# Sukikui/PTI-LDM-VAE

Measured on AMD Instinct MI355X. Metric: vae_train_images_per_sec_256x256, higher is better.
Workload: dtype fp16 forward operands + activations / bf16 backward operands + gradients, fp32 accumulate; 1 GPU; config/vae_dente_no_adv.json 256x256x1 batch 32/GPU: fwd + L1 + 1e-3*KL + bwd + all-reduce + Adam (perceptual term omitted: --perceptual times it; adversarial branch inactive before epoch 6, --adv times it); global_batch=32, parallelism=dp1

## Files before the change

include/pti_vae.h:

```cpp
#ifndef PTI_VAE_H
#define PTI_VAE_H

#include <stdint.h>

#ifdef __cplusplus
extern "C" {
#endif

typedef void* pti_stream_t;

#define PTI_ABI_VERSION 5

#define PTI_OK 0
#define PTI_EINVAL (-1)
#define PTI_EUNSUPPORTED (-2)
#define PTI_ELAUNCH (-3)

#define PTI_CONV_S1 0
#define PTI_CONV_S2PAD 1
#define PTI_CONV_UP2 2
#define PTI_CONV_ZINS 3

#define PTI_PRO_NONE 0
#define PTI_PRO_GN 1
// ... 96 lines not shown
int pti_gn_bwd_blocks(int n, int hw, int c);
int pti_gn_bwd(const void* x, const void* da, const void* dres, void* dx, const int64_t* stats,
               const float* gamma, const float* beta, float* sums, float* partials, float* dgamma,
               float* dbeta, int n, int hw, int c, int groups, float eps, int silu, int x_f16,
               pti_stream_t s);
int pti_conv_gnbwd_tiles(const pti_conv_desc* d);
int pti_conv_gnbwd_chain_supported(int cin, int cout, int ksize);
int pti_conv2d_mfma_gnbwd_chain(const void* g_in, const void* x_in, int x_in_f16, const int64_t* in_stats,
                                const float* in_gamma, const float* in_sums, void* dx_in_out, const void* w_packed,
                                const void* gx, const int64_t* gstats, const float* ggamma, const float* gbeta,
                                void* dy_out, float* gsums, const pti_conv_desc* d, int silu, pti_stream_t s);
int pti_gn_affine_grads(const float* sums, float* dgamma, float* dbeta, int n, int c, pti_stream_t s);
int pti_gn_sums_finalize_affine(const float* partials, float* sums, int n, int tiles, int row_len, const float* affine_sums,
                                float* dgamma, float* dbeta, int affine_c, pti_stream_t s);
int pti_conv2d_mfma_gnbwd(const void* dy_in, const void* w_packed, const void* gx, const int64_t* gstats,
                          const float* ggamma, const float* gbeta, void* dy_out, float* gpartials,
                          const pti_conv_desc* d, int silu, pti_stream_t s);
int pti_gn_sums_finalize(const float* partials, float* sums, int n, int tiles, int row_len,
                         pti_stream_t s);
int pti_gn_bwd_apply(const void* x, const void* dy, const void* dres, void* dx, const int64_t* stats,
                     const float* gamma, const float* beta, const float* sums, float* dgamma,
                     float* dbeta, int n, int hw, int c, int groups, float eps, int x_f16,
                     pti_stream_t s);
int pti_pool2x2_sum(const void* x, void* y, int n, int h, int w, int c, pti_stream_t s);

int pti_attention_fwd(const void* qkv, void* o, float* lse2, int b, int l, int c, pti_stream_t s);
int pti_attention_bwd(const void* qkv, const void* o, const void* dout, const float* lse2,
                      float* delta, void* dqkv, int b, int l, int c, pti_stream_t s);

int pti_latent_head_fwd(const float* h, const float* eps, const float* wm, const float* bm,
                        const float* wl, const float* bl, const float* wp, const float* bp,
                        float* mu, float* sigma, float* logvar, float* zq, int b, int hw, int l,
                        pti_stream_t s);
int pti_post_quant(const float* z_nchw, const float* wp, const float* bp, float* zq_nhwc, int b,
                   int hw, int l, pti_stream_t s);
#define PTI_POST_QUANT_BWD_MAX_BLOCKS 256
#define PTI_POST_QUANT_BWD_WS_FLOATS(l) (PTI_POST_QUANT_BWD_MAX_BLOCKS * ((l) * (l) + (l)))
int pti_post_quant_bwd(const float* dzq_nhwc, const float* z_nchw, const float* wp, float* dz_nchw,
                       float* gwp, float* gbp, float* workspace, int b, int hw, int l,
                       pti_stream_t s);
#define PTI_LATENT_BWD_MAX_BLOCKS 512
#define PTI_LATENT_BWD_WS_FLOATS(l) (PTI_LATENT_BWD_MAX_BLOCKS * 3 * ((l) * (l) + (l)))
int pti_latent_head_bwd(const float* h, const float* eps, const float* wm, const float* bm,
                        const float* wl, const float* bl, const float* wp, const float* bp,
                        const float* dzq, const float* dmu, const float* dsigma, float* dh,
                        float* gwm, float* gbm, float* gwl, float* gbl, float* gwp, float* gbp,
// ... 125 lines not shown
```

pti_ldm_vae_amd/_lib.py:

```python
from __future__ import annotations

import ctypes as C
import os

_HERE = os.path.dirname(os.path.abspath(__file__))
LIB_PATH = os.environ.get("PTI_VAE_LIB") or os.path.join(_HERE, "libpti_vae_hip.so")

def env_overrides() -> dict:
    return {k: v for k, v in sorted(os.environ.items()) if k.startswith("PTI_")}


def refuse_wrong_result_env(who: str) -> None:
    bad = [k for k in os.environ if k.startswith("PTI_") and ("DIAG" in k or k == "PTI_ALLOW_WRONG_RESULTS")]
    if bad:
        raise SystemExit(f"{who}: refusing to run with wrong-result diagnostic variable(s) set: {sorted(bad)} "
                         "(timing diagnostics live in tools/diag_skip.py)")


ABI_VERSION = 5
PTI_CONV_S1, PTI_CONV_S2PAD, PTI_CONV_UP2, PTI_CONV_ZINS = 0, 1, 2, 3
PTI_PRO_NONE, PTI_PRO_GN, PTI_PRO_GN_SILU = 0, 1, 2


class ConvDesc(C.Structure):
# ... 51 lines not shown
    "pti_gn_stats": (_I, [_P, _P, _I, _I, _I, _I, _I, _P]),
    "pti_conv2d_mfma": (_I, [_P, _P, _P, _P, _P, _P, _P, _P, _P, C.POINTER(ConvDesc), _P]),
    "pti_conv2d_mfma_saveact": (_I, [_P, _P, _P, _P, _P, _P, _P, _P, _P, _P, C.POINTER(ConvDesc), _P]),
    "pti_conv2d_direct": (_I, [_P, _P, _P, _P, _P, _P, _P, C.POINTER(ConvDesc), _P]),
    "pti_wgrad_direct": (_I, [_P, _P, _P, _P, _P, _P, _P, _P, _I, _I, _I, _I, _I, _I, _I, _I, _I, _F, _I, _I,
                              C.POINTER(_I64), _I64, _I64, _I64, _P, _I64, _P]),
    "pti_conv_wgrad_workspace_bytes": (_I64, [_I, _I, _I, _I]),
    "pti_conv_wgrad_mfma": (_I, [_P, _P, _P, _P, _P, _P, _P, _P, _I64, _I, C.POINTER(ConvDesc), _P]),
    "pti_conv_wgrad_mfma_partials": (_I, [_P, _P, _P, _P, _P, _P, _I64, C.POINTER(ConvDesc), C.POINTER(_I), _P]),
    "pti_conv_wgrad_mfma_batched": (_I, [C.POINTER(WgradJob), _I, _P, _I64, _P]),
    "pti_conv_wgrad_batched_mode": (_I, [_I, _I, _I, _I, _I]),
    "pti_direct_repack": (_I, [C.POINTER(DirectRepackTable), _P]),
    "pti_conv_wgrad_reduce": (_I, [_P, _I, _P, _P, _I, C.POINTER(ConvDesc), _P]),
    "pti_gn_bwd_blocks": (_I, [_I, _I, _I]),
    "pti_gn_bwd": (_I, [_P, _P, _P, _P, _P, _P, _P, _P, _P, _P, _P, _I, _I, _I, _I, _F, _I, _I, _P]),
    "pti_conv_gnbwd_tiles": (_I, [C.POINTER(ConvDesc)]),
    "pti_gn_sums_finalize": (_I, [_P, _P, _I, _I, _I, _P]),
    "pti_conv2d_mfma_gnbwd": (_I, [_P, _P, _P, _P, _P, _P, _P, _P, C.POINTER(ConvDesc), _I, _P]),
    "pti_conv_gnbwd_chain_supported": (_I, [_I, _I, _I]),
    "pti_conv2d_mfma_gnbwd_chain": (_I, [_P, _P, _I, _P, _P, _P, _P, _P, _P, _P, _P, _P, _P, _P, C.POINTER(ConvDesc), _I, _P]),
    "pti_gn_affine_grads": (_I, [_P, _P, _P, _I, _I, _P]),
    "pti_gn_sums_finalize_affine": (_I, [_P, _P, _I, _I, _I, _P, _P, _P, _I, _P]),
    "pti_gn_bwd_apply": (_I, [_P, _P, _P, _P, _P, _P, _P, _P, _P, _P, _I, _I, _I, _I, _F, _I, _P]),
    "pti_pool2x2_sum": (_I, [_P, _P, _I, _I, _I, _I, _P]),
    "pti_attention_fwd": (_I, [_P, _P, _P, _I, _I, _I, _P]),
    "pti_attention_bwd": (_I, [_P, _P, _P, _P, _P, _P, _I, _I, _I, _P]),
    "pti_latent_head_fwd": (_I, [_P] * 12 + [_I, _I, _I, _P]),
    "pti_post_quant": (_I, [_P, _P, _P, _P, _I, _I, _I, _P]),
    "pti_post_quant_bwd": (_I, [_P, _P, _P, _P, _P, _P, _P, _I, _I, _I, _P]),
    "pti_latent_head_bwd": (_I, [_P] * 19 + [_I, _I, _I, _P]),
    "pti_vae_loss": (_I, [_P, _P, _I64, _P, _P, _I64, _I, _P, _P, _P, _P, _P, _I, _I, _F, _P]),
    "pti_ar_vae_loss": (_I, [_P, _I, _I, _I, _P, _P, _P, _I, _P, _F, _P, _P, _P, _P]),
    "pti_pd_im2col_image": (_I, [_P, _P, _I, _I, _I, _P]),
    "pti_pd_im2col": (_I, [_P, _P, _P, _I, _I, _I, _I, _I, _I, _F, _P]),
    "pti_pd_in_stats": (_I, [_P, _P, _I, _I, _I, _F, _P]),
    "pti_pd_col2im_blocks": (_I, [_I, _I, _I]),
    "pti_pd_col2im": (_I, [_P, _P, _P, _P, _P, _I, _I, _I, _I, _I, _F, _P]),
    "pti_pd_col2im_image": (_I, [_P, _P, _I, _I, _I, _F, _I, _P]),
    "pti_pd_in_bwd_apply": (_I, [_P, _P, _P, _P, _P, _I, _I, _I, _P]),
    "pti_pd_lsgan_blocks": (_I, [_I]),
    "pti_pd_lsgan": (_I, [_P, _I, _I, _I, _F, _F, _F, _P, _P, _P]),
    "pti_pd_final_fwd": (_I, [_P, _P, _P, _P, _P, _I, _I, _I, _I, _F, _P]),
    "pti_pd_final_dgrad": (_I, [_P, _P, _P, _P, _P, _P, _I, _I, _I, _I, _F, _P]),
    "pti_pd_final_wgrad_blocks": (_I, [_I, _I, _I]),
    "pti_pd_final_wgrad": (_I, [_P, _P, _P, _P, _I, _I, _I, _I, _F, _P]),
    "pti_lpips_tap_blocks": (_I, [_I, _I]),
# ... 77 lines not shown
```

pti_ldm_vae_amd/csrc/groupnorm.hip:

```cpp
#include "pti_common.h"

namespace {

__global__ __launch_bounds__(256) void gn_stats_kernel(const bf16* __restrict__ x, stat_t* __restrict__ stats,
                                                       int HW, int C, int G, int pix_per_block, int x_f16) {
  extern __shared__ stat_t sm_q[];
  stat_t* sm = sm_q;
  const int n = blockIdx.y;
  const int tid = threadIdx.x;
  const int NC = C / 8;
  const int ppi = 256 / NC;
  const int lc = tid % NC, lp = tid / NC;
  for (int i = tid; i < 2 * G; i += 256) sm[i] = 0;
  __syncthreads();
  const int p0 = blockIdx.x * pix_per_block;
  const int p1 = min(p0 + pix_per_block, HW);
  float s[8], q[8];
#pragma unroll
  for (int j = 0; j < 8; ++j) s[j] = q[j] = 0.f;
  const bf16* base = x + (size_t)n * HW * C + lc * 8;
  int p = p0 + lp;
  for (; p + 3 * ppi < p1; p += 4 * ppi) {
    u32x4 r[4];
#pragma unroll
// ... 62 lines not shown
  int bps = cdiv(2048, n);
  int ppb = cdiv(hw, bps);
  if (ppb < 16 * ppi) ppb = 16 * ppi;
  ppb = cdiv(ppb, 4 * ppi) * 4 * ppi;
  bps = cdiv(hw, ppb);
  PTI_LAUNCH(gn_stats_kernel, dim3(bps, n), dim3(256), 2 * groups * sizeof(stat_t), (hipStream_t)s,
                     (const bf16*)x, (stat_t*)stats, hw, c, groups, ppb, x_f16);
  PTI_CHECK_LAUNCH("gn_stats");
  return PTI_OK;
}

namespace {

struct GnbArgs {
  const bf16* x; const bf16* da; const bf16* dres; bf16* dx;
  const stat_t* stats; const float* gamma; const float* beta;
  float* sums;
  float* dgamma; float* dbeta;
  int HW, C, G, silu, ppb;
  float eps, inv_cnt;
  int x_f16;
  int N;
  float* part;
};

__global__ __launch_bounds__(256) void gn_bwd_reduce_kernel(GnbArgs a) {
  extern __shared__ float sm[];
  const int n = blockIdx.y, tid = threadIdx.x;
  const int NC = a.C / 8, ppi = 256 / NC, lc = tid % NC, lp = tid / NC;
  for (int i = tid; i < 8 * a.C; i += 256) sm[i] = 0.f;
  __syncthreads();
  const int cpg = a.C / a.G;
  float sc[8], sh[8], mu[8], rs[8];
#pragma unroll
  for (int j = 0; j < 8; ++j) {
    const int ch = lc * 8 + j, g = ch / cpg;
    const float sum = stat_f(a.stats, (n * a.G + g) * 2), sq = stat_f(a.stats, (n * a.G + g) * 2 + 1);
    const float mean = sum * a.inv_cnt;
    const float rstd = rsqrtf(fmaxf(sq * a.inv_cnt - mean * mean, 0.f) + a.eps);
    mu[j] = mean; rs[j] = rstd;
    sc[j] = rstd * a.gamma[ch];
    sh[j] = a.beta[ch] - mean * sc[j];
  }
  float s1[8], s2[8];
#pragma unroll
  for (int j = 0; j < 8; ++j) s1[j] = s2[j] = 0.f;
// ... 67 lines not shown
  if (i < R) {
    const float* p = part + (size_t)n * T * R + i;
    int t = w;
    for (; t + 48 < T; t += 64) {
      const float a0 = p[(size_t)t * R], a1 = p[(size_t)(t + 16) * R], a2 = p[(size_t)(t + 32) * R], a3 = p[(size_t)(t + 48) * R];
      v += (a0 + a1) + (a2 + a3);
    }
    for (; t < T; t += 16) v += p[(size_t)t * R];
  }
  red[w][lane] = v;
  __syncthreads();
  if (w == 0 && i < R) {
    float r[16];
#pragma unroll
    for (int k = 0; k < 16; ++k) r[k] = red[k][lane];
#pragma unroll
    for (int o = 8; o > 0; o >>= 1)
#pragma unroll
      for (int k = 0; k < o; ++k) r[k] += r[k + o];
    sums[(size_t)n * R + i] = r[0];
  }
}

__global__ __launch_bounds__(256) void gn_bwd_apply_kernel(GnbArgs a) {
  const int n = blockIdx.y, tid = threadIdx.x;
  const int NC = a.C / 8, ppi = 256 / NC, lc = tid % NC, lp = tid / NC;
  const int cpg = a.C / a.G;
  const int p0 = blockIdx.x * a.ppb, p1 = min(p0 + a.ppb, a.HW);
  const size_t base = (size_t)n * a.HW * a.C + lc * 8;
  constexpr int U = 4;
  u32x4 rx[U], rd[U], rr[U];
  auto load_batch = [&](int pb) {
#pragma unroll
    for (int u = 0; u < U; ++u) {
      const int p = pb + u * ppi;
      rx[u] = rd[u] = rr[u] = u32x4{0u, 0u, 0u, 0u};
      if (p < p1) {
        rx[u] = __builtin_nontemporal_load((const u32x4*)(a.x + base + (size_t)p * a.C));
        rd[u] = __builtin_nontemporal_load((const u32x4*)(a.da + base + (size_t)p * a.C));
        if (a.dres) rr[u] = __builtin_nontemporal_load((const u32x4*)(a.dres + base + (size_t)p * a.C));
      }
    }
  };
  if (p0 + lp < p1) load_batch(p0 + lp);
  float sc[8], sh[8], mu[8], rs[8], ga[8], c1[8], c2[8];
#pragma unroll
  for (int j = 0; j < 8; ++j) {
    const int ch = lc * 8 + j, g = ch / cpg;
    const float sum = stat_f(a.stats, (n * a.G + g) * 2), sq = stat_f(a.stats, (n * a.G + g) * 2 + 1);
    const float mean = sum * a.inv_cnt;
    const float rstd = rsqrtf(fmaxf(sq * a.inv_cnt - mean * mean, 0.f) + a.eps);
    mu[j] = mean; rs[j] = rstd; ga[j] = a.gamma[ch];
    sc[j] = rstd * ga[j];
    sh[j] = a.beta[ch] - mean * sc[j];
    c1[j] = c2[j] = 0.f;
    if (cpg > 8) {
      float t1 = 0.f, t2 = 0.f;
      for (int cc = g * cpg; cc < (g + 1) * cpg; ++cc) {
        const float gm = a.gamma[cc];
        t1 += gm * a.sums[((size_t)n * a.C + cc) * 2];
        t2 += gm * a.sums[((size_t)n * a.C + cc) * 2 + 1];
      }
      c1[j] = t1 * a.inv_cnt;
      c2[j] = t2 * a.inv_cnt;
    }
  }
  if (cpg <= 8) {
    float w1[8], w2[8];
#pragma unroll
    for (int j = 0; j < 8; ++j) {
      const f32x2 sv = *(const f32x2*)(a.sums + ((size_t)n * a.C + lc * 8 + j) * 2);
      w1[j] = ga[j] * sv[0];
      w2[j] = ga[j] * sv[1];
    }
#pragma unroll
    for (int j = 0; j < 8; ++j) {
      float t1 = 0.f, t2 = 0.f;
#pragma unroll
      for (int jj = 0; jj < 8; ++jj) {
        const bool same = (jj / cpg) == (j / cpg);
        t1 += same ? w1[jj] : 0.f;
        t2 += same ? w2[jj] : 0.f;
      }
      c1[j] = t1 * a.inv_cnt;
      c2[j] = t2 * a.inv_cnt;
    }
  }
  if (blockIdx.x == 0 && n == 0) {
    for (int i = tid; i < a.C; i += 256) {
      float d1 = 0.f, d2 = 0.f;
      for (int m = 0; m < a.N; ++m) {
        d1 += a.sums[((size_t)m * a.C + i) * 2];
        d2 += a.sums[((size_t)m * a.C + i) * 2 + 1];
      }
      if (a.dbeta) a.dbeta[i] += d1;
      if (a.dgamma) a.dgamma[i] += d2;
    }
  }
  for (int pb = p0 + lp; pb < p1; pb += U * ppi) {
    if (pb != p0 + lp) load_batch(pb);
#pragma unroll
    for (int u = 0; u < U; ++u) {
      const int p = pb + u * ppi;
      float fx[8], fd[8], fr[8], o[8];
      unpack8f(rx[u], fx, a.x_f16);
      unpack8(rd[u], fd);
      unpack8(rr[u], fr);
#pragma unroll
      for (int j = 0; j < 8; ++j) {
        float dy = fd[j];
        if (a.silu) dy *= dsilu_f(fx[j] * sc[j] + sh[j]);
// ... 47 lines not shown
  if (n <= 0 || hw <= 0 || c < 8 || (c & (c - 1)) || c > 512) return 0;
  return gn_bwd_grid(n, hw, c, nullptr);
}

extern "C" int pti_gn_bwd(const void* x, const void* da, const void* dres, void* dx, const int64_t* stats,
                          const float* gamma, const float* beta, float* sums, float* partials, float* dgamma,
                          float* dbeta, int n, int hw, int c, int groups, float eps, int silu, int x_f16, pti_stream_t s) {
  if (!x || !da || !dx || !stats || !gamma || !beta || !sums || !partials) PTI_FAIL(PTI_EINVAL, "gn_bwd: null pointer");
  if (c < 8 || c > 512 || (c & (c - 1)) || groups <= 0 || c % groups) PTI_FAIL(PTI_EUNSUPPORTED, "gn_bwd: c=%d groups=%d", c, groups);
  GnbArgs a;
  a.x = (const bf16*)x; a.da = (const bf16*)da; a.dres = (const bf16*)dres; a.dx = (bf16*)dx;
  a.stats = (const stat_t*)stats; a.gamma = gamma; a.beta = beta; a.sums = sums; a.dgamma = dgamma; a.dbeta = dbeta;
  a.HW = hw; a.C = c; a.G = groups; a.silu = silu; a.eps = eps; a.x_f16 = x_f16; a.N = n;
  a.inv_cnt = 1.0f / ((float)(c / groups) * (float)hw);
  int ppb;
  const int bps = gn_bwd_grid(n, hw, c, &ppb);
  a.ppb = ppb;
  a.part = partials;
  PTI_LAUNCH(gn_bwd_reduce_kernel, dim3(bps, n), dim3(256), 8 * c * sizeof(float), (hipStream_t)s, a);
  PTI_CHECK_LAUNCH("gn_bwd_reduce");
  PTI_LAUNCH(gn_sums_finalize_kernel, dim3(cdiv(2 * c, 64), n), dim3(1024), 0, (hipStream_t)s, partials, sums,
                     bps, 2 * c, (const float*)nullptr, (float*)nullptr, (float*)nullptr, 0, 0);
  PTI_CHECK_LAUNCH("gn_sums_finalize");
  PTI_LAUNCH(gn_bwd_apply_kernel, dim3(bps, n), dim3(256), 0, (hipStream_t)s, a);
  PTI_CHECK_LAUNCH("gn_bwd_apply");
  return PTI_OK;
}

extern "C" int pti_gn_bwd_apply(const void* x, const void* dy, const void* dres, void* dx, const int64_t* stats,
                                const float* gamma, const float* beta, const float* sums, float* dgamma, float* dbeta,
                                int n, int hw, int c, int groups, float eps, int x_f16, pti_stream_t s) {
  if (!x || !dy || !dx || !stats || !gamma || !beta || !sums) PTI_FAIL(PTI_EINVAL, "gn_bwd_apply: null pointer");
  if (c < 8 || c > 2048 || (c & (c - 1)) || groups <= 0 || c % groups) PTI_FAIL(PTI_EUNSUPPORTED, "gn_bwd_apply: c=%d groups=%d", c, groups);
  GnbArgs a;
  a.x = (const bf16*)x; a.da = (const bf16*)dy; a.dres = (const bf16*)dres; a.dx = (bf16*)dx;
  a.stats = (const stat_t*)stats; a.gamma = gamma; a.beta = beta; a.sums = const_cast<float*>(sums); a.dgamma = dgamma; a.dbeta = dbeta;
  a.HW = hw; a.C = c; a.G = groups; a.silu = 0; a.eps = eps; a.x_f16 = x_f16; a.N = n;
  a.inv_cnt = 1.0f / ((float)(c / groups) * (float)hw);
  const int ppi = 256 / (c / 8);
  int bps = cdiv(2048, n);
  int ppb = cdiv(hw, bps);
  if (ppb < gnb_min_iters() * ppi) ppb = gnb_min_iters() * ppi;
  ppb = cdiv(ppb, ppi) * ppi;
  bps = cdiv(hw, ppb);
  a.ppb = ppb;
  PTI_LAUNCH(gn_bwd_apply_kernel, dim3(bps, n), dim3(256), 0, (hipStream_t)s, a);
  PTI_CHECK_LAUNCH("gn_bwd_apply");
  return PTI_OK;
}

namespace {
__global__ __launch_bounds__(256) void gn_affine_grads_kernel(const float* __restrict__ sums, float* __restrict__ dgamma,
                                                              float* __restrict__ dbeta, int n, int c) {
  const int i = blockIdx.x * 256 + threadIdx.x;
  if (i >= c) return;
  float d1 = 0.f, d2 = 0.f;
  for (int m = 0; m < n; ++m) {
    const f32x2 sv = *(const f32x2*)(sums + ((size_t)m * c + i) * 2);
    d1 += sv[0];
    d2 += sv[1];
  }
  if (dbeta) dbeta[i] += d1;
  if (dgamma) dgamma[i] += d2;
}
}

extern "C" int pti_gn_affine_grads(const float* sums, float* dgamma, float* dbeta, int n, int c, pti_stream_t s) {
  if (!sums || n <= 0 || c <= 0) PTI_FAIL(PTI_EINVAL, "gn_affine_grads: bad args");
  PTI_LAUNCH(gn_affine_grads_kernel, dim3(cdiv(c, 256)), dim3(256), 0, (hipStream_t)s, sums, dgamma, dbeta, n, c);
  PTI_CHECK_LAUNCH("gn_affine_grads");
// ... 31 lines not shown
```

pti_ldm_vae_amd/engine.py:

```python
from __future__ import annotations

import contextlib
import gc
import os
import warnings

import torch

from . import ops
from .models import autoencoderkl as M
from .ops import (BF16, F32, PTI_CONV_S1, PTI_CONV_S2PAD, PTI_CONV_UP2, PTI_CONV_ZINS, PTI_PRO_GN, PTI_PRO_GN_SILU,
                  PTI_PRO_NONE)


class _Act:

    __slots__ = ("t", "stats")

    def __init__(self, t, stats=None):
        self.t, self.stats = t, stats


def _empty(shape, like, dtype=BF16):
    return torch.empty(shape, dtype=dtype, device=like.device)
# ... 20 lines not shown
                with torch.cuda.graph(g, pool=graphs[0].pool() if graphs else None, capture_error_mode="thread_local"):
                    results.append(body(*results))
                graphs.append(g)
    except Exception as ex:
        warnings.warn(f"HIP-graph capture of {what} failed ({ex!r}); continuing with eager launches")
        torch.cuda.synchronize()
        return None
    return graphs, results


class _MfmaConv:

    def __init__(self, net, wname, bname, ksize, mode, fused_names=None, fwd_f16=True):
        self.net, self.ksize, self.mode = net, ksize, mode
        self.fwd_f16, self.f16 = fwd_f16, False
        self.wname, self.bname, self.fused = wname, bname, fused_names
        if fused_names:
            w0 = net._param_by_name[fused_names[0][0]]
            self.cout, self.cin = 3 * w0.shape[0], w0.shape[1]
        else:
            w = net._param_by_name[wname]
            self.cout, self.cin = w.shape[0], w.shape[1]
        self.wp = self.wpt = None

    def _w(self):
        if self.fused:
            o, n, _ = self.net._slots[self.fused[0][0]]
            return self.net._arena[o:o + 3 * n].view(self.cout, self.cin, 1, 1)
        return self.net._param_by_name[self.wname].data.view(self.cout, self.cin, self.ksize, self.ksize)

    def bias(self):
        if self.fused:
            o, n, _ = self.net._slots[self.fused[0][1]]
            return self.net._arena[o:o + 3 * n]
        return self.net._param_by_name[self.bname].data

    def grads(self):
        if self.fused:
            o, n, _ = self.net._slots[self.fused[0][0]]
            ob, nb, _ = self.net._slots[self.fused[0][1]]
            g = self.net.grad_arena
            return g[o:o + 3 * n], g[ob:ob + 3 * nb]
        return self.net.grad_view(self.wname).view(-1), self.net.grad_view(self.bname)

    def fwd(self, x, *, pro=PTI_PRO_NONE, norm=None, residual=None, want_stats=False, eng=None, act_out=None,
            out_dtype=None):
# ... 2 lines not shown
        y = _empty((n, ho, wo, self.cout), x.t, out_dtype or eng.act_dtype)
        st = eng.new_stats(n) if want_stats else None
        g, b = (norm.weight.data, norm.bias.data) if norm is not None else (None, None)
        ops.conv_mfma(x.t, self.wp, self.bias(), y, cout=self.cout, ksize=self.ksize, mode=self.mode, prologue=pro,
                      in_stats=x.stats if pro else None, gamma=g, beta=b, groups=eng.G, eps=eng.eps,
                      residual=residual, out_stats=st, out_groups=eng.G, act_out=act_out)
        return _Act(y, st)

    def dgrad(self, dy, *, residual=None):
        n, ho, wo, _ = dy.shape
        if self.mode == PTI_CONV_S2PAD:
            out = _empty((n, 2 * ho, 2 * wo, self.cin), dy)
            ops.conv_mfma(dy, self.wpt, None, out, cout=self.cin, ksize=3, mode=PTI_CONV_ZINS, residual=residual)
            return out
        if self.mode == PTI_CONV_UP2:
            pooled = _empty((n, ho // 2, wo // 2, self.cin), dy)
            ops.conv_mfma(dy, self.wpt, None, pooled, cout=self.cin, ksize=self.ksize, mode=PTI_CONV_S1, pool2=True)
            return pooled
        out = _empty((n, ho, wo, self.cin), dy)
        ops.conv_mfma(dy, self.wpt, None, out, cout=self.cin, ksize=self.ksize, mode=PTI_CONV_S1, residual=residual)
        return out

    def dgrad_gn(self, dy, x, norm, *, silu, dres, eng):
        g, sums = self.dgrad_gn_raw(dy, x, norm, silu=silu, eng=eng)
        return self._gn_apply(g, sums, x, norm, dres, eng)

    def _gn_apply(self, g, sums, x, norm, dres, eng):
        dx = _empty(x.t.shape, x.t)
        ops.gn_bwd_apply(x.t, g, dx, x.stats, norm.weight.data, norm.bias.data, sums,
                         norm.net.grad_view(norm.prefix + ".weight"), norm.net.grad_view(norm.prefix + ".bias"),
                         groups=eng.G, eps=eng.eps, dres=dres)
        return dx

    def dgrad_gn_raw(self, dy, x, norm, *, silu, eng):
        n, ho, wo, _ = dy.shape
        g = _empty((n, ho, wo, self.cin), dy)
        sums = eng.zeros(n * self.cin * 2)
        ops.conv_mfma_gnbwd(dy, self.wpt, x.t, x.stats, norm.weight.data, norm.bias.data, g, sums, cout=self.cin,
                            ksize=self.ksize, mode=PTI_CONV_S1, groups=eng.G, eps=eng.eps, silu=silu)
        return g, sums

    def dgrad_gn_chain(self, g_in, x_in, norm_in, sums_in, x, norm, *, silu, dres, eng):
        n, ho, wo, _ = g_in.shape
        dxin = _empty(g_in.shape, g_in)
        dyt = _empty((n, ho, wo, self.cin), g_in)
        sums = eng.zeros(n * self.cin * 2)
# ... 236 lines not shown
        last = len(eb) - 1
        for i in range(1, last - 1):
            self.enc_layers.append(self._make_layer(eb[i], f"encoder.blocks.{i}"))
        self.enc_out = _DirectConv(net, f"encoder.blocks.{last}.conv", norm_prefix=f"encoder.blocks.{last - 1}")
        db = net.decoder.blocks
        self.dec_in = _DirectConv(net, "decoder.blocks.0.conv")
        self.dec_layers = []
        last = len(db) - 1
        for i in range(1, last - 1):
            self.dec_layers.append(self._make_layer(db[i], f"decoder.blocks.{i}"))
        self.dec_out = _DirectConv(net, f"decoder.blocks.{last}.conv", norm_prefix=f"decoder.blocks.{last - 1}")
        self.mfma_convs = [c for l in self.enc_layers + self.dec_layers for c in l.convs]
        for c in self.mfma_convs:
            c.f16 = c.fwd_f16 and self.act_dtype == torch.float16
        self.direct_convs = [self.enc_in, self.enc_out, self.dec_in, self.dec_out]
        self.enc_out.pack_f16 = self.act_dtype == torch.float16
        img = os.environ.get("PTI_IMG_MFMA", "1") == "1"
        self.enc_in.img_mfma = img and 2 <= net.in_channels <= 8 and net.channels[0] % 32 == 0
        self.dec_out.img_mfma = img and 2 <= net.out_channels <= 8 and net.channels[0] % 32 == 0
        self.enc_in.pack_f16 = self.dec_out.pack_f16 = self.act_dtype == torch.float16
        self._wgrad_posts, self._wgrad_zero = [], ()
        self._flush_up = int(os.environ.get("PTI_WGRAD_FLUSH_UP", "1"))
        self.gnbwd_chain = os.environ.get("PTI_GNBWD_CHAIN", "0") == "1"
        self.Lc = net.latent_channels
        self._plist = list(net._param_by_name.values())

    def saves_activated_input(self, t) -> bool:
        return t.shape[1] * t.shape[2] >= self.save_act_min_hw

    def _make_layer(self, blk, prefix):
        if isinstance(blk, M.AEKLResBlock):
            return _ResBlock(self.net, prefix, blk)
        if isinstance(blk, M.AEKLDownsample):
            return _Resample(self.net, prefix + ".conv.conv", PTI_CONV_S2PAD, prefix + ".")
        if isinstance(blk, M.Upsample):
            return _Resample(self.net, prefix + ".postconv.conv", PTI_CONV_UP2, prefix + ".")
        if isinstance(blk, M.SpatialAttentionBlock):
            return _Attention(self.net, prefix)
        raise TypeError(f"unsupported block {type(blk)} at {prefix}")

    def new_stats(self, n):
        return self.zeros(n * self.G * 4).view(torch.int64).view(n, self.G, 2)

    def zeros(self, count):
        count = (count + 3) // 4 * 4
        pool = self._zpool
# ... 459 lines not shown
```

pti_ldm_vae_amd/ops.py:

```python
from __future__ import annotations

import ctypes as C
import os
from collections import namedtuple

import torch

from . import _lib as L
from ._lib import (PTI_CONV_S1, PTI_CONV_S2PAD, PTI_CONV_UP2, PTI_CONV_ZINS, PTI_PRO_GN, PTI_PRO_GN_SILU,
                   PTI_PRO_NONE, ConvDesc)

BF16 = torch.bfloat16
F16 = torch.float16
F32 = torch.float32
I64 = torch.int64
STAT_SCALE = 65536.0
ACT16 = (BF16, F16)
LATENT_BWD_MAX_BLOCKS = 512
VAE_LOSS_MAX_BLOCKS = 1024
POST_QUANT_BWD_MAX_BLOCKS = 256


_raw_stream = getattr(torch._C, "_cuda_getCurrentRawStream", None)
_cur_device = getattr(torch._C, "_cuda_getDevice", None)
# ... 357 lines not shown
                  ("conv wgrad (batched)", 0, 0, 0, 0, 3, "s1", len(idx)))


def gn_bwd(x, da, dx, stats, gamma, beta, sums, dgamma, dbeta, *, groups, eps=1e-6, silu=True, dres=None):
    _chk(x, ACT16, "x", 4)
    _chk(da, BF16, "da", 4)
    _chk(dx, BF16, "dx", 4)
    n, h, w, c = x.shape
    if da.shape != x.shape or dx.shape != x.shape or (dres is not None and dres.shape != x.shape):
        raise ValueError("gn_bwd: shape mismatch")
    _chk_stats(stats, n * groups * 2, "stats")
    if sums.numel() != n * c * 2:
        raise ValueError("gn_bwd: scratch sizes")
    blocks = L.lib().pti_gn_bwd_blocks(n, h * w, c)
    if blocks <= 0:
        raise ValueError(f"gn_bwd: unsupported channel count {c}")
    part = torch.empty(n * blocks * c * 2, dtype=torch.float32, device=x.device)
    L.check(L.lib().pti_gn_bwd(_ptr(x), _ptr(da), _ptr(dres), _ptr(dx), _ptr(stats), _ptr(gamma), _ptr(beta),
                               _ptr(sums), _ptr(part), _ptr(dgamma), _ptr(dbeta), n, h * w, c, groups, eps, int(silu),
                               int(x.dtype == F16), _stream()), "pti_gn_bwd")
    return dx


def conv_mfma_gnbwd(dy_in, w_packed_t, gx, gstats, ggamma, gbeta, dy_out, gsums, *, cout, ksize=3, mode=PTI_CONV_S1,
                    groups=0, eps=1e-6, silu=True):
    _chk(dy_in, BF16, "dy_in", 4)
    _chk(gx, ACT16, "gx", 4)
    _chk(dy_out, BF16, "dy_out", 4)
    n, h, w, cin = dy_in.shape
    ho, wo = conv_out_hw(h, w, mode)
    if tuple(dy_out.shape) != (n, ho, wo, cout) or gx.shape != dy_out.shape:
        raise ValueError("conv_mfma_gnbwd: shapes")
    _chk_stats(gstats, n * groups * 2, "gstats")
    if gsums.numel() != n * cout * 2 or ggamma.numel() != cout:
        raise ValueError("conv_mfma_gnbwd: GroupNorm buffers")
    d = ConvDesc(n=n, h=h, w=w, cin=cin, ho=ho, wo=wo, cout=cout, ksize=ksize, mode=mode, groups=groups, eps=eps,
                 res_f16=int(gx.dtype == F16))
    tiles = L.lib().pti_conv_gnbwd_tiles(C.byref(d))
    if tiles <= 0:
        raise ValueError("conv_mfma_gnbwd: unsupported shape")
    part = torch.empty(n * tiles * cout * 2, dtype=torch.float32, device=dy_in.device)
    prof = KERNEL_PROFILE
    rec = None if prof is None else _prof_begin(prof)
    L.check(L.lib().pti_conv2d_mfma_gnbwd(_ptr(dy_in), _ptr(w_packed_t), _ptr(gx), _ptr(gstats), _ptr(ggamma),
                                          _ptr(gbeta), _ptr(dy_out), _ptr(part), C.byref(d), int(silu), _stream()),
            "pti_conv2d_mfma_gnbwd")
    if rec is not None:
        _prof_end(rec, 2.0 * n * ho * wo * cout * cin * ksize * ksize * (0.25 if mode == PTI_CONV_ZINS else 1.0),
                  2.0 * (dy_in.numel() + 2 * dy_out.numel()),
                  ("conv dgrad+GN bwd", cin, cout, ho, wo, ksize, "zins" if mode == PTI_CONV_ZINS else "s1", n))
    L.check(L.lib().pti_gn_sums_finalize(_ptr(part), _ptr(gsums), n, tiles, 2 * cout, _stream()), "pti_gn_sums_finalize")
    return dy_out


def gnbwd_chain_supported(cin, cout, ksize, x_dtype, groups=16):
    return (x_dtype == F16 and groups > 0 and cin % groups == 0 and cin // groups >= 8
            and bool(L.lib().pti_conv_gnbwd_chain_supported(int(cin), int(cout), int(ksize))))


def conv_mfma_gnbwd_chain(g_in, x_in, in_stats, in_gamma, in_sums, dx_in, w_packed_t, gx, gstats, ggamma, gbeta, dy_out, gsums,
                          *, cout, groups, eps=1e-6, silu=True, in_dgamma=None, in_dbeta=None):
    _chk(g_in, BF16, "g_in", 4)
    _chk(x_in, ACT16, "x_in", 4)
    _chk(dx_in, BF16, "dx_in", 4)
    _chk(gx, ACT16, "gx", 4)
    _chk(dy_out, BF16, "dy_out", 4)
    n, h, w, cin = g_in.shape
    if x_in.shape != g_in.shape or dx_in.shape != g_in.shape or tuple(dy_out.shape) != (n, h, w, cout) or gx.shape != dy_out.shape:
        raise ValueError("conv_mfma_gnbwd_chain: shapes")
    _chk_stats(in_stats, n * groups * 2, "in_stats")
    _chk_stats(gstats, n * groups * 2, "gstats")
    if in_sums.numel() != n * cin * 2 or gsums.numel() != n * cout * 2 or in_gamma.numel() != cin or ggamma.numel() != cout:
        raise ValueError("conv_mfma_gnbwd_chain: GroupNorm buffers")
# ... 19 lines not shown
        L.check(L.lib().pti_gn_sums_finalize(_ptr(part), _ptr(gsums), n, tiles, 2 * cout, _stream()), "pti_gn_sums_finalize")
    return dy_out


def gn_affine_grads(sums, dgamma, dbeta, n, c):
    L.check(L.lib().pti_gn_affine_grads(_ptr(sums), _ptr(dgamma), _ptr(dbeta), int(n), int(c), _stream()), "pti_gn_affine_grads")


def gn_bwd_apply(x, dy, dx, stats, gamma, beta, sums, dgamma, dbeta, *, groups, eps=1e-6, dres=None):
    _chk(x, ACT16, "x", 4)
    _chk(dy, BF16, "dy", 4)
    _chk(dx, BF16, "dx", 4)
    n, h, w, c = x.shape
    if dy.shape != x.shape or dx.shape != x.shape or (dres is not None and dres.shape != x.shape):
        raise ValueError("gn_bwd_apply: shape mismatch")
    _chk_stats(stats, n * groups * 2, "stats")
    prof = KERNEL_PROFILE
    rec = None if prof is None else _prof_begin(prof)
    L.check(L.lib().pti_gn_bwd_apply(_ptr(x), _ptr(dy), _ptr(dres), _ptr(dx), _ptr(stats), _ptr(gamma), _ptr(beta),
                                     _ptr(sums), _ptr(dgamma), _ptr(dbeta), n, h * w, c, groups, eps,
                                     int(x.dtype == F16), _stream()), "pti_gn_bwd_apply")
    if rec is not None:
        _prof_end(rec, 8.0 * x.numel(), 2.0 * x.numel() * (4 if dres is not None else 3),
                  ("GroupNorm bwd apply", c, c, h, w, 0, "-", n))
    return dx


def pool2x2_sum(x, y):
    _chk(x, BF16, "x", 4)
    _chk(y, BF16, "y", 4)
    n, h2, w2, c = x.shape
    if tuple(y.shape) != (n, h2 // 2, w2 // 2, c) or h2 % 2 or w2 % 2:
        raise ValueError("pool2x2_sum: shapes")
    L.check(L.lib().pti_pool2x2_sum(_ptr(x), _ptr(y), n, h2 // 2, w2 // 2, c, _stream()), "pti_pool2x2_sum")
    return y


def latent_head_fwd(h, eps, wm, bm, wl, bl, wp, bp, mu, sigma, logvar, zq):
    b, hw, l = h.shape
    for t, nm in ((h, "h"), (wm, "wm"), (bm, "bm"), (wl, "wl"), (bl, "bl"), (wp, "wp"), (bp, "bp"), (mu, "mu"),
                  (sigma, "sigma"), (zq, "zq")):
        _chk(t, F32, nm)
    if mu.numel() != b * hw * l or sigma.numel() != b * hw * l or zq.numel() != b * hw * l:
        raise ValueError("latent_head_fwd: output sizes")
    if eps is not None and (eps.numel() != b * hw * l or eps.dtype != F32 or not eps.is_contiguous()):
        raise ValueError("latent_head_fwd: eps must be contiguous fp32 of the latent shape")
# ... 925 lines not shown
```

Before: 2733 images/s.

## Fold GroupNorm-backward partial sums and affine grads into the apply kernel

```diff
diff --git a/include/pti_vae.h b/include/pti_vae.h
--- a/include/pti_vae.h
+++ b/include/pti_vae.h
@@ -142,6 +142,10 @@
                      const float* gamma, const float* beta, const float* sums, float* dgamma,
                      float* dbeta, int n, int hw, int c, int groups, float eps, int x_f16,
                      pti_stream_t s);
+int pti_gn_bwd_apply_folds(int n, int hw, int c, int tiles);
+int pti_gn_bwd_apply_tiles(const void* x, const void* dy, const void* dres, void* dx, const int64_t* stats,
+                           const float* gamma, const float* beta, const float* gpartials, int tiles, float* dgamma,
+                           float* dbeta, int n, int hw, int c, int groups, float eps, int x_f16, pti_stream_t s);
 int pti_pool2x2_sum(const void* x, void* y, int n, int h, int w, int c, pti_stream_t s);
 
 int pti_attention_fwd(const void* qkv, void* o, float* lse2, int b, int l, int c, pti_stream_t s);
diff --git a/pti_ldm_vae_amd/_lib.py b/pti_ldm_vae_amd/_lib.py
--- a/pti_ldm_vae_amd/_lib.py
+++ b/pti_ldm_vae_amd/_lib.py
@@ -97,6 +97,8 @@
     "pti_gn_affine_grads": (_I, [_P, _P, _P, _I, _I, _P]),
     "pti_gn_sums_finalize_affine": (_I, [_P, _P, _I, _I, _I, _P, _P, _P, _I, _P]),
     "pti_gn_bwd_apply": (_I, [_P, _P, _P, _P, _P, _P, _P, _P, _P, _P, _I, _I, _I, _I, _F, _I, _P]),
+    "pti_gn_bwd_apply_folds": (_I, [_I, _I, _I, _I]),
+    "pti_gn_bwd_apply_tiles": (_I, [_P, _P, _P, _P, _P, _P, _P, _P, _I, _P, _P, _I, _I, _I, _I, _F, _I, _P]),
     "pti_pool2x2_sum": (_I, [_P, _P, _I, _I, _I, _I, _P]),
     "pti_attention_fwd": (_I, [_P, _P, _P, _I, _I, _I, _P]),
     "pti_attention_bwd": (_I, [_P, _P, _P, _P, _P, _P, _I, _I, _I, _P]),
diff --git a/pti_ldm_vae_amd/csrc/groupnorm.hip b/pti_ldm_vae_amd/csrc/groupnorm.hip
--- a/pti_ldm_vae_amd/csrc/groupnorm.hip
+++ b/pti_ldm_vae_amd/csrc/groupnorm.hip
@@ -108,6 +108,7 @@
   int x_f16;
   int N;
   float* part;
+  int T, bps, acols;
 };
 
 __global__ __launch_bounds__(256) void gn_bwd_reduce_kernel(GnbArgs a) {
@@ -221,13 +222,82 @@
   }
 }
 
+constexpr int GN_FOLD_MAX_TILES = 32;
+constexpr int GN_FOLD_MAX_C = 512;
+constexpr int GN_FOLD_LDS = 2048;
+
+template <int TM>
+__device__ __forceinline__ void gn_fold_load(const float* __restrict__ part, unsigned off, int T, int R, float (&q)[TM]) {
+#pragma unroll
+  for (int t = 0; t < TM; ++t) q[t] = (part + (size_t)min(t, T - 1) * R)[off];
+}
+template <int TM>
+__device__ __forceinline__ float gn_fold_sum(const float (&q)[TM], int T) {
+#pragma clang fp reassociate(off)
+  float r[16];
+#pragma unroll
+  for (int k = 0; k < 16; ++k) {
+    float v = 0.f;
+    if (k < TM) v += k < T ? q[k] : 0.f;
+    if (k + 16 < TM) v += k + 16 < T ? q[k + 16] : 0.f;
+    r[k] = v;
+  }
+#pragma unroll
+  for (int o = 8; o > 0; o >>= 1)
+#pragma unroll
+    for (int k = 0; k < o; ++k) r[k] += r[k + o];
+  return r[0];
+}
+
+template <int TM>
+__device__ __forceinline__ void gn_fold_affine(const GnbArgs& a, float* tab) {
+  const int R = 2 * a.C, tid = threadIdx.x, cpw = a.acols;
+  const int j = (blockIdx.x - a.bps) * gridDim.y + blockIdx.y;
+  if (j * cpw >= R) return;
+  const int col = tid & (cpw - 1), spp = 256 / cpw;
+#pragma clang loop unroll(disable) vectorize(disable) interleave(disable)
+  for (int m = tid / cpw; m < a.N; m += spp) {
+    float q[TM];
+    gn_fold_load(a.part, (unsigned)(m * a.T * R + j * cpw + col), a.T, R, q);
+    tab[m * cpw + col] = gn_fold_sum(q, a.T);
+  }
+  __syncthreads();
+  if (tid < cpw / 2) {
+#pragma clang fp reassociate(off)
+    const float* col = tab + 2 * tid;
+    f32x2 e = {0.f, 0.f}, o = {0.f, 0.f};
+    int m = 0;
+#pragma clang loop unroll(disable) vectorize(disable) interleave(disable)
+    for (; m + 1 < a.N; m += 2) {
+      e += *(const f32x2*)(col + m * cpw);
+      o += *(const f32x2*)(col + (m + 1) * cpw);
+    }
+    f32x2 d = e + o;
+    if (m < a.N) d += *(const f32x2*)(col + m * cpw);
+    const int i = j * (cpw / 2) + tid;
+    if (a.dbeta) a.dbeta[i] += d[0];
+    if (a.dgamma) a.dgamma[i] += d[1];
+  }
+}
+
+template <int TM>
 __global__ __launch_bounds__(256) void gn_bwd_apply_kernel(GnbArgs a) {
+  constexpr bool FOLD = TM > 0;
+  constexpr int U = 4;
+  __shared__ float fsum[FOLD ? GN_FOLD_LDS : 1];
+  if constexpr (FOLD) {
+    if ((int)blockIdx.x >= a.bps) {
+      gn_fold_affine<TM>(a, fsum);
+      return;
+    }
+  }
   const int n = blockIdx.y, tid = threadIdx.x;
   const int NC = a.C / 8, ppi = 256 / NC, lc = tid % NC, lp = tid / NC;
   const int cpg = a.C / a.G;
   const int p0 = blockIdx.x * a.ppb, p1 = min(p0 + a.ppb, a.HW);
   const size_t base = (size_t)n * a.HW * a.C + lc * 8;
-  constexpr int U = 4;
+  float q[FOLD ? TM : 1];
+  if constexpr (FOLD) gn_fold_load(a.part + (size_t)n * a.T * 2 * a.C, min(tid, 2 * a.C - 1), a.T, 2 * a.C, q);
   u32x4 rx[U], rd[U], rr[U];
   auto load_batch = [&](int pb) {
 #pragma unroll
@@ -253,18 +323,75 @@
     sc[j] = rstd * ga[j];
     sh[j] = a.beta[ch] - mean * sc[j];
     c1[j] = c2[j] = 0.f;
+    if constexpr (!FOLD)
+      if (cpg > 8) {
+        float t1 = 0.f, t2 = 0.f;
+        for (int cc = g * cpg; cc < (g + 1) * cpg; ++cc) {
+          const float gm = a.gamma[cc];
+          t1 += gm * a.sums[((size_t)n * a.C + cc) * 2];
+          t2 += gm * a.sums[((size_t)n * a.C + cc) * 2 + 1];
+        }
+        c1[j] = t1 * a.inv_cnt;
+        c2[j] = t2 * a.inv_cnt;
+      }
+  }
+  if constexpr (FOLD) {
+    if (tid < 2 * a.C) fsum[tid] = gn_fold_sum(q, a.T);
+#pragma unroll 1
+    for (int i = tid + 256; i < 2 * a.C; i += 256) {
+      gn_fold_load(a.part + (size_t)n * a.T * 2 * a.C, i, a.T, 2 * a.C, q);
+      fsum[i] = gn_fold_sum(q, a.T);
+    }
+    __syncthreads();
     if (cpg > 8) {
+#pragma unroll
+      for (int j = 0; j < 8; ++j) {
+        const int g = (lc * 8 + j) / cpg;
+        float t1 = 0.f, t2 = 0.f;
+        for (int cc = g * cpg; cc < (g + 1) * cpg; ++cc) {
+          const float gm = a.gamma[cc];
+          t1 += gm * fsum[cc * 2];
+          t2 += gm * fsum[cc * 2 + 1];
+        }
+        c1[j] = t1 * a.inv_cnt;
+        c2[j] = t2 * a.inv_cnt;
+      }
+    }
+  }
+  if (FOLD && cpg <= 8) {
+#pragma clang fp reassociate(off) contract(off)
+    float s1[8], s2[8], w1[8], w2[8];
+#pragma unroll
+    for (int j = 0; j < 8; ++j) {
+      const f32x2 sv = *(const f32x2*)(fsum + (lc * 8 + j) * 2);
+      s1[j] = sv[0];
+      s2[j] = sv[1];
+      w1[j] = ga[j] * s1[j];
+      w2[j] = ga[j] * s2[j];
+    }
+#pragma unroll
+    for (int j = 0; j < 8; ++j) {
       float t1 = 0.f, t2 = 0.f;
-      for (int cc = g * cpg; cc < (g + 1) * cpg; ++cc) {
-        const float gm = a.gamma[cc];
-        t1 += gm * a.sums[((size_t)n * a.C + cc) * 2];
-        t2 += gm * a.sums[((size_t)n * a.C + cc) * 2 + 1];
+#pragma unroll
+      for (int k = 0; k < 8; ++k) {
+        const int jj = (j == 0 && k < 2) ? 1 - k : k;
+        const bool same = (jj / cpg) == (j / cpg);
+        if (jj == j) {
+          t1 = __builtin_fmaf(ga[j], s1[j], t1);
+          t2 = __builtin_fmaf(ga[j], s2[j], t2);
+        } else if (k == 0) {
+          t1 = same ? w1[jj] : 0.f;
+          t2 = same ? w2[jj] : 0.f;
+        } else {
+          t1 = (same ? w1[jj] : 0.f) + t1;
+          t2 = (same ? w2[jj] : 0.f) + t2;
+        }
       }
       c1[j] = t1 * a.inv_cnt;
       c2[j] = t2 * a.inv_cnt;
     }
   }
-  if (cpg <= 8) {
+  if (!FOLD && cpg <= 8) {
     float w1[8], w2[8];
 #pragma unroll
     for (int j = 0; j < 8; ++j) {
@@ -285,7 +412,7 @@
       c2[j] = t2 * a.inv_cnt;
     }
   }
-  if (blockIdx.x == 0 && n == 0) {
+  if (!FOLD && blockIdx.x == 0 && n == 0) {
     for (int i = tid; i < a.C; i += 256) {
       float d1 = 0.f, d2 = 0.f;
       for (int m = 0; m < a.N; ++m) {
@@ -379,7 +506,7 @@
   PTI_LAUNCH(gn_sums_finalize_kernel, dim3(cdiv(2 * c, 64), n), dim3(1024), 0, (hipStream_t)s, partials, sums,
                      bps, 2 * c, (const float*)nullptr, (float*)nullptr, (float*)nullptr, 0, 0);
   PTI_CHECK_LAUNCH("gn_sums_finalize");
-  PTI_LAUNCH(gn_bwd_apply_kernel, dim3(bps, n), dim3(256), 0, (hipStream_t)s, a);
+  PTI_LAUNCH(gn_bwd_apply_kernel<0>, dim3(bps, n), dim3(256), 0, (hipStream_t)s, a);
   PTI_CHECK_LAUNCH("gn_bwd_apply");
   return PTI_OK;
 }
@@ -401,8 +528,56 @@
   ppb = cdiv(ppb, ppi) * ppi;
   bps = cdiv(hw, ppb);
   a.ppb = ppb;
-  PTI_LAUNCH(gn_bwd_apply_kernel, dim3(bps, n), dim3(256), 0, (hipStream_t)s, a);
+  PTI_LAUNCH(gn_bwd_apply_kernel<0>, dim3(bps, n), dim3(256), 0, (hipStream_t)s, a);
   PTI_CHECK_LAUNCH("gn_bwd_apply");
+  return PTI_OK;
+}
+
+static int gn_fold_tiles_max() {
+  const char* e = getenv("PTI_GNB_T_FOLD");
+  const int v = e ? atoi(e) : GN_FOLD_MAX_TILES;
+  return v < 0 ? 0 : v > GN_FOLD_MAX_TILES ? GN_FOLD_MAX_TILES : v;
+}
+static int gn_fold_acols(int n, int c) {
+  int cols = 8;
+  while (cols < 256 && cols * n < 2 * c) cols *= 2;
+  if (cols > 2 * c) cols = 2 * c;
+  return (long long)cols * n <= GN_FOLD_LDS ? cols : 0;
+}
+
+extern "C" int pti_gn_bwd_apply_folds(int n, int hw, int c, int tiles) {
+  if (n <= 0 || hw <= 0 || tiles <= 0 || c < 8 || (c & (c - 1)) || c > GN_FOLD_MAX_C) return 0;
+  return tiles <= gn_fold_tiles_max() && gn_fold_acols(n, c) > 0;
+}
+
+extern "C" int pti_gn_bwd_apply_tiles(const void* x, const void* dy, const void* dres, void* dx, const int64_t* stats,
+                                      const float* gamma, const float* beta, const float* partials, int tiles,
+                                      float* dgamma, float* dbeta, int n, int hw, int c, int groups, float eps, int x_f16,
+                                      pti_stream_t s) {
+  if (!x || !dy || !dx || !stats || !gamma || !beta || !partials) PTI_FAIL(PTI_EINVAL, "gn_bwd_apply_tiles: null pointer");
+  if (groups <= 0 || c % groups) PTI_FAIL(PTI_EUNSUPPORTED, "gn_bwd_apply_tiles: c=%d groups=%d", c, groups);
+  if (!pti_gn_bwd_apply_folds(n, hw, c, tiles))
+    PTI_FAIL(PTI_EUNSUPPORTED, "gn_bwd_apply_tiles: n=%d hw=%d c=%d tiles=%d does not fold", n, hw, c, tiles);
+  GnbArgs a;
+  a.x = (const bf16*)x; a.da = (const bf16*)dy; a.dres = (const bf16*)dres; a.dx = (bf16*)dx;
+  a.stats = (const stat_t*)stats; a.gamma = gamma; a.beta = beta; a.sums = nullptr; a.dgamma = dgamma; a.dbeta = dbeta;
+  a.HW = hw; a.C = c; a.G = groups; a.silu = 0; a.eps = eps; a.x_f16 = x_f16; a.N = n;
+  a.inv_cnt = 1.0f / ((float)(c / groups) * (float)hw);
+  a.part = const_cast<float*>(partials);
+  a.T = tiles;
+  int ppb;
+  a.bps = gn_bwd_grid(n, hw, c, &ppb);
+  a.ppb = ppb;
+  a.acols = gn_fold_acols(n, c);
+  const int extra = (dgamma || dbeta) ? cdiv(2 * c / a.acols, n) : 0;
+  const dim3 grid(a.bps + extra, n);
+  if (tiles <= 8)
+    PTI_LAUNCH(gn_bwd_apply_kernel<8>, grid, dim3(256), 0, (hipStream_t)s, a);
+  else if (tiles <= 16)
+    PTI_LAUNCH(gn_bwd_apply_kernel<16>, grid, dim3(256), 0, (hipStream_t)s, a);
+  else
+    PTI_LAUNCH(gn_bwd_apply_kernel<GN_FOLD_MAX_TILES>, grid, dim3(256), 0, (hipStream_t)s, a);
+  PTI_CHECK_LAUNCH("gn_bwd_apply_tiles");
   return PTI_OK;
 }
 
diff --git a/pti_ldm_vae_amd/engine.py b/pti_ldm_vae_amd/engine.py
--- a/pti_ldm_vae_amd/engine.py
+++ b/pti_ldm_vae_amd/engine.py
@@ -66,6 +66,7 @@
             w = net._param_by_name[wname]
             self.cout, self.cin = w.shape[0], w.shape[1]
         self.wp = self.wpt = None
+        self._folds = {}
 
     def _w(self):
         if self.fused:
@@ -114,6 +115,19 @@
         return out
 
     def dgrad_gn(self, dy, x, norm, *, silu, dres, eng):
+        folds = eng.gnb_fold and self._folds.get(dy.shape)
+        if folds is None:
+            folds = self._folds[dy.shape] = ops.gnbwd_folds(dy.shape, cout=self.cin, ksize=self.ksize, groups=eng.G)
+        if folds:
+            n, ho, wo, _ = dy.shape
+            g, part, tiles = ops.conv_mfma_gnbwd_tiles(dy, self.wpt, x.t, x.stats, norm.weight.data, norm.bias.data,
+                                                       _empty((n, ho, wo, self.cin), dy), cout=self.cin, ksize=self.ksize,
+                                                       mode=PTI_CONV_S1, groups=eng.G, eps=eng.eps, silu=silu)
+            dx = _empty(x.t.shape, x.t)
+            ops.gn_bwd_apply_tiles(x.t, g, dx, x.stats, norm.weight.data, norm.bias.data, part, tiles,
+                                   norm.net.grad_view(norm.prefix + ".weight"), norm.net.grad_view(norm.prefix + ".bias"),
+                                   groups=eng.G, eps=eng.eps, dres=dres)
+            return dx
         g, sums = self.dgrad_gn_raw(dy, x, norm, silu=silu, eng=eng)
         return self._gn_apply(g, sums, x, norm, dres, eng)
 
@@ -396,6 +410,7 @@
         self._wgrad_posts, self._wgrad_zero = [], ()
         self._flush_up = int(os.environ.get("PTI_WGRAD_FLUSH_UP", "1"))
         self.gnbwd_chain = os.environ.get("PTI_GNBWD_CHAIN", "0") == "1"
+        self.gnb_fold = os.environ.get("PTI_GNB_FOLD", "1") == "1"
         self.Lc = net.latent_channels
         self._plist = list(net._param_by_name.values())
 
diff --git a/pti_ldm_vae_amd/ops.py b/pti_ldm_vae_amd/ops.py
--- a/pti_ldm_vae_amd/ops.py
+++ b/pti_ldm_vae_amd/ops.py
@@ -403,8 +403,32 @@
     return dx
 
 
+def _gnbwd_desc(dy_in_shape, cout, ksize, mode, groups, eps, gx_f16):
+    n, h, w, cin = dy_in_shape
+    ho, wo = conv_out_hw(h, w, mode)
+    d = ConvDesc(n=n, h=h, w=w, cin=cin, ho=ho, wo=wo, cout=cout, ksize=ksize, mode=mode, groups=groups, eps=eps,
+                 res_f16=int(gx_f16))
+    return d, L.lib().pti_conv_gnbwd_tiles(C.byref(d))
+
+
+def gnbwd_folds(dy_in_shape, *, cout, ksize=3, mode=PTI_CONV_S1, groups=0):
+    d, tiles = _gnbwd_desc(tuple(dy_in_shape), cout, ksize, mode, groups, 1e-6, False)
+    return tiles > 0 and bool(L.lib().pti_gn_bwd_apply_folds(d.n, d.ho * d.wo, cout, tiles))
+
+
+def conv_mfma_gnbwd_tiles(dy_in, w_packed_t, gx, gstats, ggamma, gbeta, dy_out, *, cout, ksize=3, mode=PTI_CONV_S1, groups=0,
+                          eps=1e-6, silu=True):
+    return _conv_mfma_gnbwd(dy_in, w_packed_t, gx, gstats, ggamma, gbeta, dy_out, None, cout, ksize, mode, groups, eps, silu)
+
+
 def conv_mfma_gnbwd(dy_in, w_packed_t, gx, gstats, ggamma, gbeta, dy_out, gsums, *, cout, ksize=3, mode=PTI_CONV_S1,
                     groups=0, eps=1e-6, silu=True):
+    if gsums is None:
+        raise ValueError("conv_mfma_gnbwd: gsums")
+    return _conv_mfma_gnbwd(dy_in, w_packed_t, gx, gstats, ggamma, gbeta, dy_out, gsums, cout, ksize, mode, groups, eps, silu)
+
+
+def _conv_mfma_gnbwd(dy_in, w_packed_t, gx, gstats, ggamma, gbeta, dy_out, gsums, cout, ksize, mode, groups, eps, silu):
     _chk(dy_in, BF16, "dy_in", 4)
     _chk(gx, ACT16, "gx", 4)
     _chk(dy_out, BF16, "dy_out", 4)
@@ -413,11 +437,9 @@
     if tuple(dy_out.shape) != (n, ho, wo, cout) or gx.shape != dy_out.shape:
         raise ValueError("conv_mfma_gnbwd: shapes")
     _chk_stats(gstats, n * groups * 2, "gstats")
-    if gsums.numel() != n * cout * 2 or ggamma.numel() != cout:
+    if (gsums is not None and gsums.numel() != n * cout * 2) or ggamma.numel() != cout:
         raise ValueError("conv_mfma_gnbwd: GroupNorm buffers")
-    d = ConvDesc(n=n, h=h, w=w, cin=cin, ho=ho, wo=wo, cout=cout, ksize=ksize, mode=mode, groups=groups, eps=eps,
-                 res_f16=int(gx.dtype == F16))
-    tiles = L.lib().pti_conv_gnbwd_tiles(C.byref(d))
+    d, tiles = _gnbwd_desc((n, h, w, cin), cout, ksize, mode, groups, eps, gx.dtype == F16)
     if tiles <= 0:
         raise ValueError("conv_mfma_gnbwd: unsupported shape")
     part = torch.empty(n * tiles * cout * 2, dtype=torch.float32, device=dy_in.device)
@@ -430,6 +452,8 @@
         _prof_end(rec, 2.0 * n * ho * wo * cout * cin * ksize * ksize * (0.25 if mode == PTI_CONV_ZINS else 1.0),
                   2.0 * (dy_in.numel() + 2 * dy_out.numel()),
                   ("conv dgrad+GN bwd", cin, cout, ho, wo, ksize, "zins" if mode == PTI_CONV_ZINS else "s1", n))
+    if gsums is None:
+        return dy_out, part, tiles
     L.check(L.lib().pti_gn_sums_finalize(_ptr(part), _ptr(gsums), n, tiles, 2 * cout, _stream()), "pti_gn_sums_finalize")
     return dy_out
 
@@ -495,6 +519,28 @@
                                      int(x.dtype == F16), _stream()), "pti_gn_bwd_apply")
     if rec is not None:
         _prof_end(rec, 8.0 * x.numel(), 2.0 * x.numel() * (4 if dres is not None else 3),
+                  ("GroupNorm bwd apply", c, c, h, w, 0, "-", n))
+    return dx
+
+
+def gn_bwd_apply_tiles(x, dy, dx, stats, gamma, beta, part, tiles, dgamma, dbeta, *, groups, eps=1e-6, dres=None):
+    _chk(x, ACT16, "x", 4)
+    _chk(dy, BF16, "dy", 4)
+    _chk(dx, BF16, "dx", 4)
+    _chk(part, F32, "part")
+    n, h, w, c = x.shape
+    if dy.shape != x.shape or dx.shape != x.shape or (dres is not None and dres.shape != x.shape):
+        raise ValueError("gn_bwd_apply_tiles: shape mismatch")
+    if tiles <= 0 or part.numel() != n * tiles * c * 2:
+        raise ValueError("gn_bwd_apply_tiles: partial rows")
+    _chk_stats(stats, n * groups * 2, "stats")
+    prof = KERNEL_PROFILE
+    rec = None if prof is None else _prof_begin(prof)
+    L.check(L.lib().pti_gn_bwd_apply_tiles(_ptr(x), _ptr(dy), _ptr(dres), _ptr(dx), _ptr(stats), _ptr(gamma), _ptr(beta),
+                                           _ptr(part), int(tiles), _ptr(dgamma), _ptr(dbeta), n, h * w, c, groups, eps,
+                                           int(x.dtype == F16), _stream()), "pti_gn_bwd_apply_tiles")
+    if rec is not None:
+        _prof_end(rec, 8.0 * x.numel(), 2.0 * x.numel() * (4 if dres is not None else 3) + 4.0 * part.numel(),
                   ("GroupNorm bwd apply", c, c, h, w, 0, "-", n))
     return dx
 
```

After: 2748 images/s, median of 6. About the same (+0.6%).
